# Ray0089/geometric-aware-dense-matching

Measured on AMD Instinct MI355X. Metric: rgbd_crops_per_sec_geomatch_fwd, higher is better.
Workload: dtype bf16x3/f32acc

## Files before the change

geometric_aware_dense_matching_amd/csrc/gdm_conv.hip:

```cpp
#include "gdm_common.h"
#include <math.h>
#include <limits.h>
#include <stdlib.h>

namespace {

constexpr int ROWB = 512;
constexpr int CV_PIX = 256;
constexpr int CV_CO = 128;
constexpr int CV_PANEL = CV_CO * ROWB;
#ifndef GDM_CONV16_PF
#define GDM_CONV16_PF 2
#endif

__device__ __forceinline__ void split8(const float* v, unsigned (&hi)[4], unsigned (&lo)[4])
{
#pragma unroll
    for (int j = 0; j < 4; ++j) gdm_split2(v[2 * j], v[2 * j + 1], hi[j], lo[j]);
}

__global__ __launch_bounds__(256) void conv_pack_act_kernel(const float* __restrict__ x, int C, int H, int W,
                                                            unsigned char* __restrict__ out)
{
    __shared__ float t[128][65];
// ... 57 lines not shown
#define GDM_CONV16_LATE 1
#endif
constexpr int MF_NPH = GDM_CONV_NPH;
constexpr int MF_WPIX = 16 * MF_NPH;
constexpr int MF_WAVES = CV_PIX / MF_WPIX;
constexpr int MF_THREADS = MF_WAVES * 64;
constexpr int conv_lds_bytes(int NCB)
{
    const int panels = 2 * NCB * 16 * ROWB, tiles = CV_PIX * (NCB * 16 + 4) * 4;
    return panels > tiles ? panels : tiles;
}
constexpr int LDS_MAX = 160 * 1024;
static_assert(conv_lds_bytes(8) == 135168 && conv_lds_bytes(4) == 69632 && conv_lds_bytes(9) == 151552 && conv_lds_bytes(8) >= 2 * CV_PANEL,
              "at least what every launch site passes");

template <int ACT, bool HAS_RES, int TAPS = 9, bool PIXMAJOR = false, int NKS = 8, int NCB = 8, int WV = MF_WAVES, bool GADD = false>
__global__ __launch_bounds__(MF_THREADS) void conv_mfma16_kernel(const unsigned char* __restrict__ xpk, const unsigned char* __restrict__ wpk,
                                                                 const float* __restrict__ scale, const float* __restrict__ shift,
                                                                 const float* __restrict__ res, int B, int Cin, int Cout, int H, int W,
                                                                 float* __restrict__ out, const int32_t* __restrict__ rowidx = nullptr,
                                                                 const int32_t* __restrict__ tile_co0 = nullptr,
                                                                 unsigned char* __restrict__ outpk = nullptr, int stride = 1,
                                                                 long wbstride = 0,
                                                                 const int32_t* __restrict__ gidx = nullptr,
                                                                 const float* __restrict__ gt = nullptr, int gn = 0,
                                                                 int gt_lds = 0)
{
    extern __shared__ __attribute__((aligned(16))) unsigned char smem[];
    constexpr int NS = NKS / 2;
    constexpr int UG = (NCB % 2 == 0) ? 2 : 3;
    constexpr int NPR = NCB / UG;
    constexpr int PANEL = NCB * 16 * ROWB;
    constexpr int TST = NCB * 16 + 4;
    static_assert(NCB == 8 || (NCB == 4 && !PIXMAJOR) || (NCB == 9 && !PIXMAJOR && WV == 8),
                  "64-channel tiles: NCHW / packed output only; 144-channel tiles: NCHW fp32 output only (no packed output: a tile straddles 128-channel chunks)");
    constexpr int NPH = MF_NPH;
    const int tid = threadIdx.x, lane = tid & 63;
    const int wave = __builtin_amdgcn_readfirstlane(tid >> 6);
    const int l16 = lane & 15, kg = lane >> 4;
    const int nchunk = (Cin + 127) / 128;
    const int npanel = TAPS * nchunk;
    const int hw = H * W;
    const long ptot = rowidx ? (long)B : (long)B * hw;
    const unsigned bx = blockIdx.x, by = blockIdx.y;
    const long pix0 = (long)bx * (WV * MF_WPIX) + wave * MF_WPIX;
    const int co0 = tile_co0 ? __builtin_amdgcn_readfirstlane(tile_co0[bx]) : by * (NCB * 16);
    const long pc = min(pix0, ptot - MF_WPIX);
    const int b = (int)(pc / hw);
    const int prem = (int)(pc - (long)b * hw);
    const int Wi = W * stride;
    const long plane = (long)(H * stride + 2) * (Wi + 2);
    const long oplane = (long)(H + 2) * (W + 2);
    const __amdgpu_buffer_rsrc_t xr = __builtin_amdgcn_make_buffer_rsrc(const_cast<unsigned char*>(xpk), (short)0, 0x7ffffff0, 0x00020000);
    int avoff[NPH];
#pragma unroll
    for (int ph = 0; ph < NPH; ++ph) {
        const int pr = prem + 16 * ph;
        const int yy = pr / W, xx = pr - yy * W;
        const long pixbase = rowidx ? (long)max(rowidx[pc + l16 + 16 * ph], 0) : (long)(yy * stride) * (Wi + 2) + (long)(xx + l16) * stride;
        avoff[ph] = (int)(((long)kg * plane + pixbase) * 16);
    }

    gdm_u32x4 ahi[NS][NPH], alo[NS][NPH];
    struct Pan { int chunk, ky, kx; };
    auto pan_next = [&](Pan p) -> Pan {
        if (TAPS == 1) { ++p.chunk; return p; }
        if (++p.kx == 3) { p.kx = 0; if (++p.ky == 3) { p.ky = 0; ++p.chunk; } }
        return p;
    };
    const int a_base = (int)(((long)(rowidx ? 0 : b) * nchunk * 32) * plane * 16);
    const int a_chunk = (int)(32 * plane * 16), a_rowb = (Wi + 2) * 16;
    auto pan_a = [&](Pan p) -> int { return a_base + p.chunk * a_chunk + p.ky * a_rowb + p.kx * 16; };
    const int sstride = (int)(4 * plane * 16);
    const int lostride = (int)(16 * plane * 16);
    auto load_a = [&](int r, int S) {
#pragma unroll
        for (int ph = 0; ph < NPH; ++ph) {
            ahi[S][ph] = __builtin_bit_cast(gdm_u32x4, __builtin_amdgcn_raw_buffer_load_b128(xr, avoff[ph], r + S * sstride, 0));
            alo[S][ph] = __builtin_bit_cast(gdm_u32x4, __builtin_amdgcn_raw_buffer_load_b128(xr, avoff[ph], r + S * sstride + lostride, 0));
        }
    };
    constexpr int THREADS = WV * 64, WGPIX = WV * MF_WPIX;
    constexpr int HS = (NCB * 512 / THREADS) / 2;
    gdm_u32x4 stage[HS];
    const __amdgpu_buffer_rsrc_t wr = __builtin_amdgcn_make_buffer_rsrc(const_cast<unsigned char*>(wpk), (short)0, 0x7ffffff0, 0x00020000);
    const int w_base = (wbstride ? (int)(((long)bx * WGPIX / hw) * wbstride) : 0) + co0 * ROWB;
    const int w_panel = ((Cout + 127) & ~127) * ROWB;
    auto pan_w = [&](Pan p) -> int { return w_base + ((TAPS == 1) ? p.chunk : (p.ky * 3 + p.kx) * nchunk + p.chunk) * w_panel; };
    auto stage_load = [&](int src, int half) {
#pragma unroll
        for (int i = 0; i < HS; ++i)
            stage[i] = __builtin_bit_cast(gdm_u32x4, __builtin_amdgcn_raw_buffer_load_b128(wr, tid * 16, src + (half * HS + i) * THREADS * 16, 0));
    };
    auto stage_store = [&](int buf, int half) {
        unsigned char* base = smem + buf * PANEL;
#pragma unroll
        for (int i = 0; i < HS; ++i) {
            const int g = (half * HS + i) * THREADS + tid;
            *reinterpret_cast<gdm_u32x4*>(base + gdm_swz<ROWB>(g >> 5, g & 31)) = stage[i];
        }
    };
    constexpr bool GLDS = WV == 8;
    constexpr int NPIECE = PANEL / 1024 / 8;
    int glds_voff = 0;
    if (GLDS) {
        const int hrow = lane >> 5, sl = lane & 31;
        const int col15 = (2 * wave + hrow) & 15;
        glds_voff = wave * 1024 + hrow * 512 + (((sl & 16) | ((sl ^ col15) & 15)) << 4);
    }
    typedef __attribute__((address_space(3))) void* lds_void_ptr;
    auto stage_glds = [&](int src, int buf) {
#pragma unroll
        for (int i = 0; i < NPIECE; ++i)
            __builtin_amdgcn_raw_ptr_buffer_load_lds(wr, (lds_void_ptr)(smem + buf * PANEL + (i * 8 + wave) * 1024), 16, glds_voff, src + i * 8192, 0, 0);
    };

    gdm_f32x4 acc[NPH][NCB];
#pragma unroll
    for (int ph = 0; ph < NPH; ++ph)
#pragma unroll
        for (int cb = 0; cb < NCB; ++cb)
#pragma unroll
            for (int i = 0; i < 4; ++i) acc[ph][cb][i] = 0.f;

    constexpr int LATE = GDM_CONV16_LATE < NS ? GDM_CONV16_LATE : NS;
    Pan pcur = {0, (TAPS == 1) ? 1 : 0, (TAPS == 1) ? 1 : 0};
    if (GLDS) {
        stage_glds(pan_w(pcur), 0);
    } else {
        stage_load(pan_w(pcur), 0);
        stage_store(0, 0);
        stage_load(pan_w(pcur), 1);
        stage_store(0, 1);
    }
    int rcur = pan_a(pcur);
#pragma unroll
    for (int S = 0; S < NS - LATE; ++S) load_a(rcur, S);
    Pan pnxt = npanel > 1 ? pan_next(pcur) : pcur;
    int rnext = pan_a(pnxt), wnext = pan_w(pnxt);
    for (int it = 0; it < npanel; ++it) {
        __syncthreads();
        const bool more = it + 1 < npanel;
        const unsigned char* base = smem + (it & 1) * PANEL;
        constexpr int PF = GDM_CONV16_PF;
        constexpr int NU = NPR * NS;
        gdm_u32x4 fh[PF + 1][UG], fl[PF + 1][UG];
        auto frag_load = [&](int un) {
            const int S = un / NPR, pr = un % NPR, slot = un % (PF + 1);
#pragma unroll
            for (int j = 0; j < UG; ++j) {
                const int col = (UG * pr + j) * 16 + l16;
                fh[slot][j] = *reinterpret_cast<const gdm_u32x4*>(base + gdm_swz<ROWB>(col, 4 * S + kg));
                fl[slot][j] = *reinterpret_cast<const gdm_u32x4*>(base + gdm_swz<ROWB>(col, 16 + 4 * S + kg));
            }
        };
#pragma unroll
        for (int un = 0; un < PF; ++un) frag_load(un);
#pragma unroll
        for (int u = 0; u < NU; ++u) {
            const int S = u / NPR, pr = u % NPR, slot = u % (PF + 1);
            if (u + PF < NU) frag_load(u + PF);
#pragma unroll
            for (int ph = 0; ph < NPH; ++ph) {
                const gdm_bf16x8 ah = __builtin_bit_cast(gdm_bf16x8, ahi[S][ph]);
                const gdm_bf16x8 al = __builtin_bit_cast(gdm_bf16x8, alo[S][ph]);
#pragma unroll
                for (int j = 0; j < UG; ++j) {
                    gdm_f32x4 c = acc[ph][UG * pr + j];
                    c = __builtin_amdgcn_mfma_f32_16x16x32_bf16(ah, __builtin_bit_cast(gdm_bf16x8, fl[slot][j]), c, 0, 0, 0);
                    c = __builtin_amdgcn_mfma_f32_16x16x32_bf16(al, __builtin_bit_cast(gdm_bf16x8, fh[slot][j]), c, 0, 0, 0);
                    c = __builtin_amdgcn_mfma_f32_16x16x32_bf16(ah, __builtin_bit_cast(gdm_bf16x8, fh[slot][j]), c, 0, 0, 0);
                    acc[ph][UG * pr + j] = c;
                }
            }
            if (pr == NPR - 1 && S < NS - LATE) load_a(rnext, S);
            if (!GLDS && u == NU / 2 && more) {
                stage_store((it + 1) & 1, 0);
                stage_load(wnext, 1);
            }
            if (u == 0) {
                if (more) { if (GLDS) stage_glds(wnext, (it + 1) & 1); else stage_load(wnext, 0); }
#pragma unroll
                for (int S2 = NS - LATE; S2 < NS; ++S2) load_a(rcur, S2);
            }
#pragma unroll
            for (int i = 0; i < 3 * UG * NPH; ++i) {
                __builtin_amdgcn_sched_group_barrier(0x008, 1, 0);
                if (u + PF < NU && (i % NPH) == 0 && i < 2 * UG * NPH) __builtin_amdgcn_sched_group_barrier(0x100, 1, 0);
            }
            __builtin_amdgcn_sched_barrier(0);
        }
        if (!GLDS && more) stage_store((it + 1) & 1, 1);
        rcur = rnext;
        if (it + 2 < npanel) pnxt = pan_next(pnxt);
        rnext = pan_a(pnxt);
        wnext = pan_w(pnxt);
    }

    if (pix0 >= ptot) return;
    if (PIXMAJOR) {
#pragma unroll
        for (int cb = 0; cb < NCB; ++cb) {
            const int co = co0 + cb * 16 + l16;
            if (co >= Cout) continue;
            const float sc = scale ? scale[co] : 1.f, sh = shift ? shift[co] : 0.f;
            const int ocol = tile_co0 ? cb * 16 + l16 : co;
            const int ostride = tile_co0 ? CV_CO : Cout;
#pragma unroll
            for (int ph = 0; ph < NPH; ++ph)
#pragma unroll
                for (int r = 0; r < 4; ++r) {
                    float v = acc[ph][cb][r] * sc + sh;
                    if (ACT == 1) v = fmaxf(v, 0.f);
                    out[(pix0 + 16 * ph + 4 * kg + r) * ostride + ocol] = v;
                }
        }
        return;
    }
    float gtv[GADD ? NPH : 1][GADD ? NCB : 1][4], gsc[GADD ? NCB : 1], gsh[GADD ? NCB : 1];
    int gsrc[GADD ? NPH : 1][4];
    if constexpr (GADD) {
#pragma unroll
        for (int ph = 0; ph < NPH; ++ph) {
            const int4 i4 = *reinterpret_cast<const int4*>(gidx + (long)b * hw + prem + 16 * ph + 4 * kg);
            gsrc[ph][0] = min(max(i4.x, 0), gn - 1);
            gsrc[ph][1] = min(max(i4.y, 0), gn - 1);
            gsrc[ph][2] = min(max(i4.z, 0), gn - 1);
            gsrc[ph][3] = min(max(i4.w, 0), gn - 1);
        }
#pragma unroll
        for (int cb = 0; cb < NCB; ++cb) {
            const int cl = min(co0 + cb * 16 + l16, Cout - 1);
            gsc[cb] = scale[cl];
            gsh[cb] = shift[cl];
        }
        if (gt_lds) {
            float* ts = reinterpret_cast<float*>(smem + gt_lds);
            for (int r = wave; r < NCB * 16; r += WV) {
                const float* tp = gt + ((long)b * Cout + min(co0 + r, Cout - 1)) * gn;
                for (int c = lane; c < gn; c += 64) ts[r * (gn + 1) + c] = tp[c];
            }
        } else {
#pragma unroll
            for (int cb = 0; cb < NCB; ++cb) {
                const float* tp = gt + ((long)b * Cout + min(co0 + cb * 16 + l16, Cout - 1)) * gn;
#pragma unroll
                for (int ph = 0; ph < NPH; ++ph)
#pragma unroll
                    for (int j = 0; j < 4; ++j) gtv[ph][cb][j] = tp[gsrc[ph][j]];
            }
        }
    }
    float* tl = reinterpret_cast<float*>(smem) + wave * MF_WPIX * TST;
    if (outpk || (GADD && gt_lds)) __syncthreads();
    if constexpr (GADD) {
        if (gt_lds) {
            const float* ts = reinterpret_cast<const float*>(smem + gt_lds);
#pragma unroll
            for (int cb = 0; cb < NCB; ++cb)
#pragma unroll
                for (int ph = 0; ph < NPH; ++ph)
#pragma unroll
                    for (int j = 0; j < 4; ++j) gtv[ph][cb][j] = ts[(cb * 16 + l16) * (gn + 1) + gsrc[ph][j]];
        }
    }
#pragma unroll
    for (int cb = 0; cb < NCB; ++cb) {
        const int co = co0 + cb * 16 + l16;
        const bool live = co < Cout;
        float sc, sh;
        if constexpr (GADD) { sc = gsc[cb]; sh = gsh[cb]; }
        else { sc = (live && scale) ? scale[co] : 1.f; sh = (live && shift) ? shift[co] : 0.f; }
        float* op = out ? out + ((long)b * Cout + (live ? co : 0)) * hw + prem : nullptr;
        const float* rp = (HAS_RES && live) ? res + ((long)b * Cout + co) * hw + prem : nullptr;
#pragma unroll
        for (int ph = 0; ph < NPH; ++ph) {
            const int poff = 16 * ph + 4 * kg;
            float v[4];
            if constexpr (GADD) {
#pragma unroll
                for (int j = 0; j < 4; ++j) {
                    const float x = acc[ph][cb][j] * 1.f + 0.f;
                    v[j] = (x + gtv[ph][cb][j]) * sc + sh;
                }
            } else {
#pragma unroll
                for (int j = 0; j < 4; ++j) v[j] = acc[ph][cb][j] * sc + sh;
            }
            if (HAS_RES && live) {
                const float4 r4 = *reinterpret_cast<const float4*>(rp + poff);
                v[0] += r4.x; v[1] += r4.y; v[2] += r4.z; v[3] += r4.w;
            }
            if (ACT == 1) {
#pragma unroll
                for (int j = 0; j < 4; ++j) v[j] = fmaxf(v[j], 0.f);
            }
            if (op && live) *reinterpret_cast<float4*>(op + poff) = make_float4(v[0], v[1], v[2], v[3]);
            if (outpk) {
#pragma unroll
                for (int j = 0; j < 4; ++j) tl[(poff + j) * TST + cb * 16 + l16] = live ? v[j] : 0.f;
            }
        }
    }
    if (outpk) {
        __builtin_amdgcn_fence(__ATOMIC_ACQ_REL, "wavefront");
        const int lr = lane & 31, h = lane >> 5;
        const int ochunks = (Cout + 127) / 128;
        const int ochunk = co0 / 128;
#pragma unroll
        for (int half = 0; half < MF_WPIX / 32; ++half) {
            const int pp = prem + 32 * half + lr;
            const int yy = pp / W, xx = pp - yy * W;
            unsigned char* ob = outpk + (((long)(b * ochunks + ochunk) * 32) * oplane + (long)(yy + 1) * (W + 2) + xx + 1) * 16;
            const float* row = tl + (32 * half + lr) * TST;
#pragma unroll
            for (int it = 0; it < NCB; ++it) {
                const int ql = 2 * it + h;
                if (co0 + ql * 8 >= Cout) continue;
                const int q = (co0 % 128) / 8 + ql;
                const float4 a0 = *reinterpret_cast<const float4*>(row + ql * 8);
                const float4 a1 = *reinterpret_cast<const float4*>(row + ql * 8 + 4);
                const float v[8] = {a0.x, a0.y, a0.z, a0.w, a1.x, a1.y, a1.z, a1.w};
                unsigned hi[4], lo[4];
                split8(v, hi, lo);
                *reinterpret_cast<uint4*>(ob + (long)q * oplane * 16) = make_uint4(hi[0], hi[1], hi[2], hi[3]);
                *reinterpret_cast<uint4*>(ob + (long)(16 + q) * oplane * 16) = make_uint4(lo[0], lo[1], lo[2], lo[3]);
            }
        }
    }
}

struct ConvArgs {
    const void *xpk = nullptr, *wpk = nullptr;
    const float *scale = nullptr, *shift = nullptr, *res = nullptr;
    int B = 0, Cin = 0, Cout = 0, H = 0, W = 0;
    float* out = nullptr;
    const int32_t *rowidx = nullptr, *tile_co0 = nullptr;
    void* outpk = nullptr;
    int stride = 1;
    long wbstride = 0;
    const int32_t* gidx = nullptr;
    const float* gt = nullptr;
    int gn = 0, gt_lds = 0;
    const char* who = "conv_mfma16_kernel";
};

static long mul_sat(long a, long b)
{
    long r;
    return (a < 0 || b < 0 || __builtin_mul_overflow(a, b, &r)) ? LONG_MAX : r;
}

template <int ACT, bool RES, int TAPS, bool PM, int NKS, int NCB, int WV, bool GADD>
int conv_launch(dim3 grid, int smem, hipStream_t s, const ConvArgs& a)
{
    const long chunks = (a.Cin + 127) / 128;
    const long xbytes = mul_sat(mul_sat(a.rowidx ? 1 : a.B, mul_sat((long)a.H * a.stride + 2, (long)a.W * a.stride + 2)), chunks * ROWB);
    const long wpanels = mul_sat(TAPS * chunks, (((long)a.Cout + 127) & ~127L) * ROWB);
    const long wlead = a.wbstride ? mul_sat(a.B - 1, a.wbstride) : 0;
    const long wbytes = wlead > LONG_MAX - wpanels ? LONG_MAX : wlead + wpanels;
    GDM_CHECK_ARG(xbytes < (1L << 31) && wbytes < (1L << 31),
                  "%s: packed operands must stay below 2 GiB (activations %ld bytes, weights %ld bytes)", a.who, xbytes, wbytes);
    GDM_CHECK_ARG((((uintptr_t)a.xpk | (uintptr_t)a.wpk) & 15) == 0,
                  "%s: the packed operands must be 16-byte aligned (xpk %p, wpk %p)", a.who, a.xpk, a.wpk);
    GDM_CHECK_ARG((((uintptr_t)a.res | (uintptr_t)a.out) & 15) == 0, "%s: res and out must be 16-byte aligned (res %p, out %p)", a.who,
                  (const void*)a.res, (const void*)a.out);
    constexpr auto kernel = conv_mfma16_kernel<ACT, RES, TAPS, PM, NKS, NCB, WV, GADD>;
    gdm_allow_lds<kernel>(GADD ? LDS_MAX : conv_lds_bytes(NCB));
    hipLaunchKernelGGL(kernel, grid, dim3(WV * 64), smem, s, (const unsigned char*)a.xpk, (const unsigned char*)a.wpk, a.scale, a.shift, a.res,
                       a.B, a.Cin, a.Cout, a.H, a.W, a.out, a.rowidx, a.tile_co0, (unsigned char*)a.outpk, a.stride, a.wbstride, a.gidx, a.gt,
                       a.gn, a.gt_lds);
    return 0;
}

}

namespace {
template <int CHAIN>
__global__ __launch_bounds__(512) void mfma_probe_kernel(int iters, float* __restrict__ sink)
{
    const int lane = threadIdx.x & 63;
    gdm_f32x4 acc[8];
#pragma unroll
    for (int i = 0; i < 8; ++i) acc[i] = gdm_f32x4{0.f, 0.f, 0.f, 0.f};
    const unsigned seed = 0x3f803f80u + (unsigned)lane;
    gdm_u32x4 av = {seed, seed ^ 1u, seed ^ 2u, seed ^ 3u}, bv = {seed ^ 4u, seed ^ 5u, seed ^ 6u, seed ^ 7u};
    const gdm_bf16x8 a = __builtin_bit_cast(gdm_bf16x8, av), b = __builtin_bit_cast(gdm_bf16x8, bv);
    for (int it = 0; it < iters; it += CHAIN) {
#pragma unroll
// ... 178 lines not shown
    return gdm_launch_status("gemm_grouped_kernel");
}

extern "C" int gdm_conv1x1_packed_wb_hip(const void* xpk, const void* wpk, long w_bstride, int B, int Cin, int Cout, int H, int W, float* out,
                                         void* stream)
{
    GDM_CHECK_ARG(xpk && wpk && out, "gdm_conv1x1_packed_wb_hip: NULL pointer");
    GDM_CHECK_ARG(B >= 1 && Cin >= 128 && Cin % 128 == 0 && Cout >= 1, "gdm_conv1x1_packed_wb_hip: Cin=%d Cout=%d (Cin a multiple of 128)", Cin, Cout);
    GDM_CHECK_ARG(W % 32 == 0 && H >= 1 && (H * W) % CV_PIX == 0, "gdm_conv1x1_packed_wb_hip: W=%d must be a multiple of 32 and H*W=%d of %d",
                  W, H * W, CV_PIX);
    GDM_CHECK_ARG(w_bstride >= 0 && w_bstride % 16 == 0, "gdm_conv1x1_packed_wb_hip: w_bstride=%ld", w_bstride);
    const long ptot = (long)B * H * W;
    const dim3 grid(gdm_cdiv(ptot, CV_PIX), gdm_cdiv(Cout, CV_CO));
    ConvArgs a{xpk, wpk, nullptr, nullptr, nullptr, B, Cin, Cout, H, W, out};
    a.wbstride = w_bstride; a.who = "gdm_conv1x1_packed_wb_hip";
    if (int refused = conv_launch<0, false, 1, false, 8, 8, MF_WAVES, false>(grid, 2 * CV_PANEL, (hipStream_t)stream, a)) return refused;
    return gdm_launch_status("conv1x1_bf16x3_kernel (per-image weights)");
}

static int conv1x1_launch(const void* xpk, const void* wpk, const float* scale, const float* shift,
                          int B, int Cin, int Cout, int H, int W, int stride, int act, int pixel_major, float* out, void* stream,
                          const char* who)
{
    GDM_CHECK_ARG(stride == 1 || stride == 2, "%s: stride=%d (1 or 2)", who, stride);
    GDM_CHECK_ARG(xpk && wpk && out, "%s: NULL pointer", who);
    GDM_CHECK_ARG(B >= 1 && cin_ok(Cin) && Cout >= 1, "%s: Cin=%d Cout=%d (Cin a multiple of 128, or 64)", who, Cin, Cout);
    GDM_CHECK_ARG(Cin != 64 || !pixel_major, "%s: Cin=64 is built for the NCHW output only", who);
    GDM_CHECK_ARG(W % 32 == 0 && H >= 1 && (H * W) % MF_WPIX == 0,
                  "%s: W=%d must be a multiple of 32 and H*W=%d of %d", who, W, H * W, MF_WPIX);
    GDM_CHECK_ARG(act == 0 || act == 1, "%s: act=%d", who, act);
    const long ptot = (long)B * H * W;
    const unsigned ptiles = gdm_cdiv(ptot, CV_PIX);
    hipStream_t s = (hipStream_t)stream;
    ConvArgs a{xpk, wpk, scale, shift, nullptr, B, Cin, Cout, H, W, out};
    a.stride = stride; a.who = who;
    int refused = 0;
    if (Cin != 64 && !pixel_major && stride == 1 && Cout % 144 == 0) {
        const long r128 = gdm_cdiv((long)ptiles * gdm_cdiv(Cout, 128), 256) * 128, r144 = gdm_cdiv((long)ptiles * (Cout / 144), 256) * 144;
        if (r144 < r128) {
            const dim3 grid9(ptiles, Cout / 144);
            gdm_dispatch_int<2>(act, [&](auto A) {
                refused = conv_launch<decltype(A)::value, false, 1, false, 8, 9, MF_WAVES, false>(grid9, conv_lds_bytes(9), s, a);
            });
            if (refused) return refused;
            return gdm_launch_status("conv1x1_bf16x3_kernel (144-channel tiles)");
        }
    }
    const bool narrow = Cin != 64 && !pixel_major && narrow_tiles(ptiles, Cout);
    const unsigned ctiles = gdm_cdiv(Cout, narrow ? 64 : CV_CO);
    const dim3 grid(ptiles, ctiles);
    gdm_dispatch_int<2>(act, [&](auto A) {
        constexpr int ACT = decltype(A)::value;
        if (Cin == 64)
            refused = conv_launch<ACT, false, 1, false, 4, 8, MF_WAVES, false>(grid, 2 * CV_PANEL, s, a);
        else if (narrow)
            refused = conv_launch<ACT, false, 1, false, 8, 4, MF_WAVES, false>(grid, 2 * 64 * ROWB, s, a);
        else
            gdm_dispatch_bool(pixel_major != 0, [&](auto P) {
                refused = conv_launch<ACT, false, 1, decltype(P)::value, 8, 8, MF_WAVES, false>(grid, 2 * CV_PANEL, s, a);
            });
    });
    if (refused) return refused;
    return gdm_launch_status(narrow ? "conv1x1_bf16x3_kernel (64-channel tiles)" : "conv1x1_bf16x3_kernel");
}

extern "C" int gdm_conv1x1_packed_hip(const void* xpk, const void* wpk, const float* scale, const float* shift,
                                      int B, int Cin, int Cout, int H, int W, int act, int pixel_major, float* out, void* stream)
{
    return conv1x1_launch(xpk, wpk, scale, shift, B, Cin, Cout, H, W, 1, act, pixel_major, out, stream, "gdm_conv1x1_packed_hip");
}

extern "C" int gdm_conv1x1_strided_hip(const void* xpk, const void* wpk, const float* scale, const float* shift,
                                       int B, int Cin, int Cout, int H, int W, int stride, int act, float* out, void* stream)
{
// ... 38 lines not shown
```

include/gdm.h:

```cpp
#ifndef GDM_H
#define GDM_H

#include <stddef.h>
#include <stdint.h>

#ifdef __cplusplus
extern "C" {
#endif

#define GDM_EINVAL (-1)
#define GDM_ENOMEM (-2)

const char* gdm_last_error(void);
int gdm_version(void);


void gdm_knn_batch(const float* batch_data, size_t batch_size, size_t npts, size_t dim,
                   const float* queries, size_t nqueries, size_t K, long* batch_indices);

int gdm_knn_batch_hip(const float* support, const float* query, int B, int S, int Q, int K,
                      int32_t* idx, float* d2, void* stream);

typedef struct gdm_knn_job {
    const float* support;
// ... 321 lines not shown
int gdm_stem_hip(const float* x, const void* wpk, const float* scale, const float* shift, int B, int H, int W, float* out,
                 void* out_packed, void* stream);

size_t gdm_wgrad_x_bytes(int B, int Cin, int H, int W);
size_t gdm_wgrad_go_bytes(int B, int Cout, int H, int W);
int gdm_wgrad_pack_x_hip(const float* x, int B, int Cin, int H, int W, void* out, void* stream);
int gdm_wgrad_pack_go_hip(const float* go, int B, int Cout, int H, int W, void* out, void* stream);
size_t gdm_wgrad_x1_bytes(int B, int Cin, int P);
int gdm_wgrad_pack_x1_hip(const float* x, int B, int Cin, int P, void* out, void* stream);
int gdm_mfma_probe_hip(int blocks, int iters, int chain, float* sink, void* stream);
int gdm_mfma_probe_lds_hip(int blocks, int iters, int rpu, float* sink, void* stream);
int gdm_wgrad_direct_hip(const float* go, long go_bstride, const float* x, long x_bstride, int B, int Cout, int Cin, int P,
                         int nsplit, float* partial, float* bias_partial, void* stream);
int gdm_conv1x1_packed_wb_hip(const void* xpk, const void* wpk, long w_bstride, int B, int Cin, int Cout, int H, int W, float* out,
                              void* stream);

typedef struct gdm_copy_job {
    void* dst;
    const void* src;
    int64_t sb, s1, s2;
    int32_t B, R1, R2, E;
} gdm_copy_job;
#define GDM_COPY_MAX_JOBS 16
int gdm_copy_jobs_hip(const gdm_copy_job* jobs , int njobs, void* stream);

int gdm_mssd_mspd_hip(const double* RT_est, const double* RT_gt, const double* pts, const double* sym_R, const double* sym_t,
                      const double* K, int k_per_instance, int n, int M, int S, double* err, double* mssd, double* mspd,
                      int32_t* best_sym_mssd, int32_t* best_sym_mspd, void* stream);
int gdm_render_depth_hip(const void* verts, int verts_f64, const int32_t* faces, const double* RT, const double* K, int k_per_instance,
                         int n, int V, int F, int H, int W, double near, int keep_inf, float* depth, void* stream);
// ... 25 lines not shown
```

Before: 5271.

## Make 1x1 conv kernels persistent, prefetching the next tile's operands across tiles

The 1x1 MFMA conv sites now launch a persistent grid sized to CU count times workgroups per CU. Each workgroup loops over output tiles with a grid stride. While finishing the last panel of one tile, it prefetches the next tile's activation fragments and weight panel, so the pipeline fill is not paid per tile and launch/tail overhead drops. In exchange there are fewer workgroups in flight, more register pressure from the extra tile state, and a possible load imbalance at the tail.

```diff
diff --git a/geometric_aware_dense_matching_amd/csrc/gdm_conv.hip b/geometric_aware_dense_matching_amd/csrc/gdm_conv.hip
--- a/geometric_aware_dense_matching_amd/csrc/gdm_conv.hip
+++ b/geometric_aware_dense_matching_amd/csrc/gdm_conv.hip
@@ -2,6 +2,7 @@
 #include <math.h>
 #include <limits.h>
 #include <stdlib.h>
+#include <atomic>
 
 namespace {
 
@@ -95,7 +96,8 @@
 static_assert(conv_lds_bytes(8) == 135168 && conv_lds_bytes(4) == 69632 && conv_lds_bytes(9) == 151552 && conv_lds_bytes(8) >= 2 * CV_PANEL,
               "at least what every launch site passes");
 
-template <int ACT, bool HAS_RES, int TAPS = 9, bool PIXMAJOR = false, int NKS = 8, int NCB = 8, int WV = MF_WAVES, bool GADD = false>
+template <int ACT, bool HAS_RES, int TAPS = 9, bool PIXMAJOR = false, int NKS = 8, int NCB = 8, int WV = MF_WAVES, bool GADD = false,
+          bool LOOP = false>
 __global__ __launch_bounds__(MF_THREADS) void conv_mfma16_kernel(const unsigned char* __restrict__ xpk, const unsigned char* __restrict__ wpk,
                                                                  const float* __restrict__ scale, const float* __restrict__ shift,
                                                                  const float* __restrict__ res, int B, int Cin, int Cout, int H, int W,
@@ -105,8 +107,10 @@
                                                                  long wbstride = 0,
                                                                  const int32_t* __restrict__ gidx = nullptr,
                                                                  const float* __restrict__ gt = nullptr, int gn = 0,
-                                                                 int gt_lds = 0)
-{
+                                                                 int gt_lds = 0,
+                                                                 unsigned ntiles = 0, unsigned ptiles = 1)
+{
+    static_assert(!LOOP || (TAPS == 1 && WV == 8 && !GADD), "the tile loop is built for the plain 1x1 sites: one tap, weight panels by LDS-DMA");
     extern __shared__ __attribute__((aligned(16))) unsigned char smem[];
     constexpr int NS = NKS / 2;
     constexpr int UG = (NCB % 2 == 0) ? 2 : 3;
@@ -123,24 +127,43 @@
     const int npanel = TAPS * nchunk;
     const int hw = H * W;
     const long ptot = rowidx ? (long)B : (long)B * hw;
-    const unsigned bx = blockIdx.x, by = blockIdx.y;
-    const long pix0 = (long)bx * (WV * MF_WPIX) + wave * MF_WPIX;
-    const int co0 = tile_co0 ? __builtin_amdgcn_readfirstlane(tile_co0[bx]) : by * (NCB * 16);
-    const long pc = min(pix0, ptot - MF_WPIX);
-    const int b = (int)(pc / hw);
-    const int prem = (int)(pc - (long)b * hw);
     const int Wi = W * stride;
     const long plane = (long)(H * stride + 2) * (Wi + 2);
     const long oplane = (long)(H + 2) * (W + 2);
+    constexpr int THREADS = WV * 64, WGPIX = WV * MF_WPIX;
+    struct Tile {
+        long pix0;
+        int co0, b, prem;
+        int a_base, w_base;
+        int avoff[NPH];
+    };
+    auto tile_at = [&](unsigned bx, unsigned by) -> Tile {
+        Tile T;
+        T.pix0 = (long)bx * WGPIX + wave * MF_WPIX;
+        T.co0 = tile_co0 ? __builtin_amdgcn_readfirstlane(tile_co0[bx]) : by * (NCB * 16);
+        const long pc = min(T.pix0, ptot - MF_WPIX);
+        T.b = (int)(pc / hw);
+        T.prem = (int)(pc - (long)T.b * hw);
+#pragma unroll
+        for (int ph = 0; ph < NPH; ++ph) {
+            const int pr = T.prem + 16 * ph;
+            const int yy = pr / W, xx = pr - yy * W;
+            const long pixbase = rowidx ? (long)max(rowidx[pc + l16 + 16 * ph], 0) : (long)(yy * stride) * (Wi + 2) + (long)(xx + l16) * stride;
+            T.avoff[ph] = (int)(((long)kg * plane + pixbase) * 16);
+        }
+        T.a_base = (int)(((long)(rowidx ? 0 : T.b) * nchunk * 32) * plane * 16);
+        T.w_base = (wbstride ? (int)(((long)bx * WGPIX / hw) * wbstride) : 0) + T.co0 * ROWB;
+        return T;
+    };
+    unsigned t = blockIdx.x;
+    auto next_of = [&](unsigned tt) -> unsigned { return tt + gridDim.x < ntiles ? tt + gridDim.x : tt; };
+    Tile cur = LOOP ? tile_at(t % ptiles, t / ptiles) : tile_at(blockIdx.x, blockIdx.y);
+    unsigned tn = LOOP ? next_of(t) : t;
+    Tile nxt_tile = LOOP ? tile_at(tn % ptiles, tn / ptiles) : Tile{};
+    Tile& nxt = LOOP ? nxt_tile : cur;
+    const long& pix0 = cur.pix0;
+    const int &co0 = cur.co0, &b = cur.b, &prem = cur.prem;
     const __amdgpu_buffer_rsrc_t xr = __builtin_amdgcn_make_buffer_rsrc(const_cast<unsigned char*>(xpk), (short)0, 0x7ffffff0, 0x00020000);
-    int avoff[NPH];
-#pragma unroll
-    for (int ph = 0; ph < NPH; ++ph) {
-        const int pr = prem + 16 * ph;
-        const int yy = pr / W, xx = pr - yy * W;
-        const long pixbase = rowidx ? (long)max(rowidx[pc + l16 + 16 * ph], 0) : (long)(yy * stride) * (Wi + 2) + (long)(xx + l16) * stride;
-        avoff[ph] = (int)(((long)kg * plane + pixbase) * 16);
-    }
 
     gdm_u32x4 ahi[NS][NPH], alo[NS][NPH];
     struct Pan { int chunk, ky, kx; };
@@ -149,25 +172,22 @@
         if (++p.kx == 3) { p.kx = 0; if (++p.ky == 3) { p.ky = 0; ++p.chunk; } }
         return p;
     };
-    const int a_base = (int)(((long)(rowidx ? 0 : b) * nchunk * 32) * plane * 16);
     const int a_chunk = (int)(32 * plane * 16), a_rowb = (Wi + 2) * 16;
-    auto pan_a = [&](Pan p) -> int { return a_base + p.chunk * a_chunk + p.ky * a_rowb + p.kx * 16; };
+    auto pan_a = [&](const Tile& T, Pan p) -> int { return T.a_base + p.chunk * a_chunk + p.ky * a_rowb + p.kx * 16; };
     const int sstride = (int)(4 * plane * 16);
     const int lostride = (int)(16 * plane * 16);
-    auto load_a = [&](int r, int S) {
+    auto load_a = [&](const int* avoff, int r, int S) {
 #pragma unroll
         for (int ph = 0; ph < NPH; ++ph) {
             ahi[S][ph] = __builtin_bit_cast(gdm_u32x4, __builtin_amdgcn_raw_buffer_load_b128(xr, avoff[ph], r + S * sstride, 0));
             alo[S][ph] = __builtin_bit_cast(gdm_u32x4, __builtin_amdgcn_raw_buffer_load_b128(xr, avoff[ph], r + S * sstride + lostride, 0));
         }
     };
-    constexpr int THREADS = WV * 64, WGPIX = WV * MF_WPIX;
     constexpr int HS = (NCB * 512 / THREADS) / 2;
     gdm_u32x4 stage[HS];
     const __amdgpu_buffer_rsrc_t wr = __builtin_amdgcn_make_buffer_rsrc(const_cast<unsigned char*>(wpk), (short)0, 0x7ffffff0, 0x00020000);
-    const int w_base = (wbstride ? (int)(((long)bx * WGPIX / hw) * wbstride) : 0) + co0 * ROWB;
     const int w_panel = ((Cout + 127) & ~127) * ROWB;
-    auto pan_w = [&](Pan p) -> int { return w_base + ((TAPS == 1) ? p.chunk : (p.ky * 3 + p.kx) * nchunk + p.chunk) * w_panel; };
+    auto pan_w = [&](const Tile& T, Pan p) -> int { return T.w_base + ((TAPS == 1) ? p.chunk : (p.ky * 3 + p.kx) * nchunk + p.chunk) * w_panel; };
     auto stage_load = [&](int src, int half) {
 #pragma unroll
         for (int i = 0; i < HS; ++i)
@@ -197,216 +217,236 @@
     };
 
     gdm_f32x4 acc[NPH][NCB];
-#pragma unroll
-    for (int ph = 0; ph < NPH; ++ph)
-#pragma unroll
-        for (int cb = 0; cb < NCB; ++cb)
-#pragma unroll
-            for (int i = 0; i < 4; ++i) acc[ph][cb][i] = 0.f;
-
     constexpr int LATE = GDM_CONV16_LATE < NS ? GDM_CONV16_LATE : NS;
-    Pan pcur = {0, (TAPS == 1) ? 1 : 0, (TAPS == 1) ? 1 : 0};
+    const Pan pfirst = {0, (TAPS == 1) ? 1 : 0, (TAPS == 1) ? 1 : 0};
     if (GLDS) {
-        stage_glds(pan_w(pcur), 0);
+        stage_glds(pan_w(cur, pfirst), 0);
     } else {
-        stage_load(pan_w(pcur), 0);
+        stage_load(pan_w(cur, pfirst), 0);
         stage_store(0, 0);
-        stage_load(pan_w(pcur), 1);
+        stage_load(pan_w(cur, pfirst), 1);
         stage_store(0, 1);
     }
-    int rcur = pan_a(pcur);
-#pragma unroll
-    for (int S = 0; S < NS - LATE; ++S) load_a(rcur, S);
-    Pan pnxt = npanel > 1 ? pan_next(pcur) : pcur;
-    int rnext = pan_a(pnxt), wnext = pan_w(pnxt);
-    for (int it = 0; it < npanel; ++it) {
-        __syncthreads();
-        const bool more = it + 1 < npanel;
-        const unsigned char* base = smem + (it & 1) * PANEL;
-        constexpr int PF = GDM_CONV16_PF;
-        constexpr int NU = NPR * NS;
-        gdm_u32x4 fh[PF + 1][UG], fl[PF + 1][UG];
-        auto frag_load = [&](int un) {
-            const int S = un / NPR, pr = un % NPR, slot = un % (PF + 1);
-#pragma unroll
-            for (int j = 0; j < UG; ++j) {
-                const int col = (UG * pr + j) * 16 + l16;
-                fh[slot][j] = *reinterpret_cast<const gdm_u32x4*>(base + gdm_swz<ROWB>(col, 4 * S + kg));
-                fl[slot][j] = *reinterpret_cast<const gdm_u32x4*>(base + gdm_swz<ROWB>(col, 16 + 4 * S + kg));
+#pragma unroll
+    for (int S = 0; S < NS - LATE; ++S) load_a(cur.avoff, pan_a(cur, pfirst), S);
+    unsigned pcnt = 0;
+    for (;;) {
+        const bool last_tile = !LOOP || tn == t;
+#pragma unroll
+        for (int ph = 0; ph < NPH; ++ph)
+#pragma unroll
+            for (int cb = 0; cb < NCB; ++cb)
+#pragma unroll
+                for (int i = 0; i < 4; ++i) acc[ph][cb][i] = 0.f;
+        int rcur = pan_a(cur, pfirst);
+        Pan pnxt = npanel > 1 ? pan_next(pfirst) : pfirst;
+        int rnext = (LOOP && npanel == 1) ? pan_a(nxt, pfirst) : pan_a(cur, pnxt);
+        int wnext = (LOOP && npanel == 1) ? pan_w(nxt, pfirst) : pan_w(cur, pnxt);
+        for (int it = 0; it < npanel; ++it, ++pcnt) {
+            __syncthreads();
+            const bool more = it + 1 < npanel;
+            const bool wmore = more || !last_tile;
+            const unsigned char* base = smem + (pcnt & 1) * PANEL;
+            int avnext[NPH];
+#pragma unroll
+            for (int ph = 0; ph < NPH; ++ph) avnext[ph] = (LOOP && !more) ? nxt.avoff[ph] : cur.avoff[ph];
+            constexpr int PF = GDM_CONV16_PF;
+            constexpr int NU = NPR * NS;
+            gdm_u32x4 fh[PF + 1][UG], fl[PF + 1][UG];
+            auto frag_load = [&](int un) {
+                const int S = un / NPR, pr = un % NPR, slot = un % (PF + 1);
+#pragma unroll
+                for (int j = 0; j < UG; ++j) {
+                    const int col = (UG * pr + j) * 16 + l16;
+                    fh[slot][j] = *reinterpret_cast<const gdm_u32x4*>(base + gdm_swz<ROWB>(col, 4 * S + kg));
+                    fl[slot][j] = *reinterpret_cast<const gdm_u32x4*>(base + gdm_swz<ROWB>(col, 16 + 4 * S + kg));
+                }
+            };
+#pragma unroll
+            for (int un = 0; un < PF; ++un) frag_load(un);
+#pragma unroll
+            for (int u = 0; u < NU; ++u) {
+                const int S = u / NPR, pr = u % NPR, slot = u % (PF + 1);
+                if (u + PF < NU) frag_load(u + PF);
+#pragma unroll
+                for (int ph = 0; ph < NPH; ++ph) {
+                    const gdm_bf16x8 ah = __builtin_bit_cast(gdm_bf16x8, ahi[S][ph]);
+                    const gdm_bf16x8 al = __builtin_bit_cast(gdm_bf16x8, alo[S][ph]);
+#pragma unroll
+                    for (int j = 0; j < UG; ++j) {
+                        gdm_f32x4 c = acc[ph][UG * pr + j];
+                        c = __builtin_amdgcn_mfma_f32_16x16x32_bf16(ah, __builtin_bit_cast(gdm_bf16x8, fl[slot][j]), c, 0, 0, 0);
+                        c = __builtin_amdgcn_mfma_f32_16x16x32_bf16(al, __builtin_bit_cast(gdm_bf16x8, fh[slot][j]), c, 0, 0, 0);
+                        c = __builtin_amdgcn_mfma_f32_16x16x32_bf16(ah, __builtin_bit_cast(gdm_bf16x8, fh[slot][j]), c, 0, 0, 0);
+                        acc[ph][UG * pr + j] = c;
+                    }
+                }
+                if (pr == NPR - 1 && S < NS - LATE) load_a(avnext, rnext, S);
+                if (!GLDS && u == NU / 2 && more) {
+                    stage_store((pcnt + 1) & 1, 0);
+                    stage_load(wnext, 1);
+                }
+                if (u == 0) {
+                    if (wmore) { if (GLDS) stage_glds(wnext, (pcnt + 1) & 1); else stage_load(wnext, 0); }
+#pragma unroll
+                    for (int S2 = NS - LATE; S2 < NS; ++S2) load_a(cur.avoff, rcur, S2);
+                }
+#pragma unroll
+                for (int i = 0; i < 3 * UG * NPH; ++i) {
+                    __builtin_amdgcn_sched_group_barrier(0x008, 1, 0);
+                    if (u + PF < NU && (i % NPH) == 0 && i < 2 * UG * NPH) __builtin_amdgcn_sched_group_barrier(0x100, 1, 0);
+                }
+                __builtin_amdgcn_sched_barrier(0);
             }
-        };
-#pragma unroll
-        for (int un = 0; un < PF; ++un) frag_load(un);
-#pragma unroll
-        for (int u = 0; u < NU; ++u) {
-            const int S = u / NPR, pr = u % NPR, slot = u % (PF + 1);
-            if (u + PF < NU) frag_load(u + PF);
-#pragma unroll
-            for (int ph = 0; ph < NPH; ++ph) {
-                const gdm_bf16x8 ah = __builtin_bit_cast(gdm_bf16x8, ahi[S][ph]);
-                const gdm_bf16x8 al = __builtin_bit_cast(gdm_bf16x8, alo[S][ph]);
-#pragma unroll
-                for (int j = 0; j < UG; ++j) {
-                    gdm_f32x4 c = acc[ph][UG * pr + j];
-                    c = __builtin_amdgcn_mfma_f32_16x16x32_bf16(ah, __builtin_bit_cast(gdm_bf16x8, fl[slot][j]), c, 0, 0, 0);
-                    c = __builtin_amdgcn_mfma_f32_16x16x32_bf16(al, __builtin_bit_cast(gdm_bf16x8, fh[slot][j]), c, 0, 0, 0);
-                    c = __builtin_amdgcn_mfma_f32_16x16x32_bf16(ah, __builtin_bit_cast(gdm_bf16x8, fh[slot][j]), c, 0, 0, 0);
-                    acc[ph][UG * pr + j] = c;
-                }
-            }
-            if (pr == NPR - 1 && S < NS - LATE) load_a(rnext, S);
-            if (!GLDS && u == NU / 2 && more) {
-                stage_store((it + 1) & 1, 0);
-                stage_load(wnext, 1);
-            }
-            if (u == 0) {
-                if (more) { if (GLDS) stage_glds(wnext, (it + 1) & 1); else stage_load(wnext, 0); }
-#pragma unroll
-                for (int S2 = NS - LATE; S2 < NS; ++S2) load_a(rcur, S2);
-            }
-#pragma unroll
-            for (int i = 0; i < 3 * UG * NPH; ++i) {
-                __builtin_amdgcn_sched_group_barrier(0x008, 1, 0);
-                if (u + PF < NU && (i % NPH) == 0 && i < 2 * UG * NPH) __builtin_amdgcn_sched_group_barrier(0x100, 1, 0);
-            }
-            __builtin_amdgcn_sched_barrier(0);
+            if (!GLDS && more) stage_store((pcnt + 1) & 1, 1);
+            rcur = rnext;
+            if (it + 2 < npanel) pnxt = pan_next(pnxt);
+            const bool over = LOOP && it + 2 >= npanel;
+            rnext = over ? pan_a(nxt, pfirst) : pan_a(cur, pnxt);
+            wnext = over ? pan_w(nxt, pfirst) : pan_w(cur, pnxt);
         }
-        if (!GLDS && more) stage_store((it + 1) & 1, 1);
-        rcur = rnext;
-        if (it + 2 < npanel) pnxt = pan_next(pnxt);
-        rnext = pan_a(pnxt);
-        wnext = pan_w(pnxt);
-    }
-
-    if (pix0 >= ptot) return;
-    if (PIXMAJOR) {
-#pragma unroll
-        for (int cb = 0; cb < NCB; ++cb) {
-            const int co = co0 + cb * 16 + l16;
-            if (co >= Cout) continue;
-            const float sc = scale ? scale[co] : 1.f, sh = shift ? shift[co] : 0.f;
-            const int ocol = tile_co0 ? cb * 16 + l16 : co;
-            const int ostride = tile_co0 ? CV_CO : Cout;
-#pragma unroll
-            for (int ph = 0; ph < NPH; ++ph)
-#pragma unroll
-                for (int r = 0; r < 4; ++r) {
-                    float v = acc[ph][cb][r] * sc + sh;
-                    if (ACT == 1) v = fmaxf(v, 0.f);
-                    out[(pix0 + 16 * ph + 4 * kg + r) * ostride + ocol] = v;
-                }
-        }
-        return;
-    }
-    float gtv[GADD ? NPH : 1][GADD ? NCB : 1][4], gsc[GADD ? NCB : 1], gsh[GADD ? NCB : 1];
-    int gsrc[GADD ? NPH : 1][4];
-    if constexpr (GADD) {
-#pragma unroll
-        for (int ph = 0; ph < NPH; ++ph) {
-            const int4 i4 = *reinterpret_cast<const int4*>(gidx + (long)b * hw + prem + 16 * ph + 4 * kg);
-            gsrc[ph][0] = min(max(i4.x, 0), gn - 1);
-            gsrc[ph][1] = min(max(i4.y, 0), gn - 1);
-            gsrc[ph][2] = min(max(i4.z, 0), gn - 1);
-            gsrc[ph][3] = min(max(i4.w, 0), gn - 1);
-        }
-#pragma unroll
-        for (int cb = 0; cb < NCB; ++cb) {
-            const int cl = min(co0 + cb * 16 + l16, Cout - 1);
-            gsc[cb] = scale[cl];
-            gsh[cb] = shift[cl];
-        }
-        if (gt_lds) {
-            float* ts = reinterpret_cast<float*>(smem + gt_lds);
-            for (int r = wave; r < NCB * 16; r += WV) {
-                const float* tp = gt + ((long)b * Cout + min(co0 + r, Cout - 1)) * gn;
-                for (int c = lane; c < gn; c += 64) ts[r * (gn + 1) + c] = tp[c];
+
+        if (!LOOP && pix0 >= ptot) return;
+        const bool wlive = !LOOP || pix0 < ptot;
+        int lane = tid & 63;
+        if constexpr (LOOP) asm volatile("" : "+v"(lane));
+        const int l16 = lane & 15, kg = lane >> 4;
+        if constexpr (PIXMAJOR) {
+#pragma unroll
+            for (int cb = 0; cb < NCB; ++cb) {
+                const int co = co0 + cb * 16 + l16;
+                if (co >= Cout) continue;
+                const float sc = scale ? scale[co] : 1.f, sh = shift ? shift[co] : 0.f;
+                const int ocol = tile_co0 ? cb * 16 + l16 : co;
+                const int ostride = tile_co0 ? CV_CO : Cout;
+#pragma unroll
+                for (int ph = 0; ph < NPH; ++ph)
+#pragma unroll
+                    for (int r = 0; r < 4; ++r) {
+                        float v = acc[ph][cb][r] * sc + sh;
+                        if (ACT == 1) v = fmaxf(v, 0.f);
+                        if (wlive) out[(pix0 + 16 * ph + 4 * kg + r) * ostride + ocol] = v;
+                    }
             }
         } else {
+            float gtv[GADD ? NPH : 1][GADD ? NCB : 1][4], gsc[GADD ? NCB : 1], gsh[GADD ? NCB : 1];
+            int gsrc[GADD ? NPH : 1][4];
+            if constexpr (GADD) {
+#pragma unroll
+                for (int ph = 0; ph < NPH; ++ph) {
+                    const int4 i4 = *reinterpret_cast<const int4*>(gidx + (long)b * hw + prem + 16 * ph + 4 * kg);
+                    gsrc[ph][0] = min(max(i4.x, 0), gn - 1);
+                    gsrc[ph][1] = min(max(i4.y, 0), gn - 1);
+                    gsrc[ph][2] = min(max(i4.z, 0), gn - 1);
+                    gsrc[ph][3] = min(max(i4.w, 0), gn - 1);
+                }
+#pragma unroll
+                for (int cb = 0; cb < NCB; ++cb) {
+                    const int cl = min(co0 + cb * 16 + l16, Cout - 1);
+                    gsc[cb] = scale[cl];
+                    gsh[cb] = shift[cl];
+                }
+                if (gt_lds) {
+                    float* ts = reinterpret_cast<float*>(smem + gt_lds);
+                    for (int r = wave; r < NCB * 16; r += WV) {
+                        const float* tp = gt + ((long)b * Cout + min(co0 + r, Cout - 1)) * gn;
+                        for (int c = lane; c < gn; c += 64) ts[r * (gn + 1) + c] = tp[c];
+                    }
+                } else {
+#pragma unroll
+                    for (int cb = 0; cb < NCB; ++cb) {
+                        const float* tp = gt + ((long)b * Cout + min(co0 + cb * 16 + l16, Cout - 1)) * gn;
+#pragma unroll
+                        for (int ph = 0; ph < NPH; ++ph)
+#pragma unroll
+                            for (int j = 0; j < 4; ++j) gtv[ph][cb][j] = tp[gsrc[ph][j]];
+                    }
+                }
+            }
+            float* tl = reinterpret_cast<float*>(smem) + wave * MF_WPIX * TST;
+            if (outpk || (GADD && gt_lds)) __syncthreads();
+            if constexpr (GADD) {
+                if (gt_lds) {
+                    const float* ts = reinterpret_cast<const float*>(smem + gt_lds);
+#pragma unroll
+                    for (int cb = 0; cb < NCB; ++cb)
+#pragma unroll
+                        for (int ph = 0; ph < NPH; ++ph)
+#pragma unroll
+                            for (int j = 0; j < 4; ++j) gtv[ph][cb][j] = ts[(cb * 16 + l16) * (gn + 1) + gsrc[ph][j]];
+                }
+            }
 #pragma unroll
             for (int cb = 0; cb < NCB; ++cb) {
-                const float* tp = gt + ((long)b * Cout + min(co0 + cb * 16 + l16, Cout - 1)) * gn;
-#pragma unroll
-                for (int ph = 0; ph < NPH; ++ph)
-#pragma unroll
-                    for (int j = 0; j < 4; ++j) gtv[ph][cb][j] = tp[gsrc[ph][j]];
+                const int co = co0 + cb * 16 + l16;
+                const bool live = co < Cout;
+                float sc, sh;
+                if constexpr (GADD) { sc = gsc[cb]; sh = gsh[cb]; }
+                else { sc = (live && scale) ? scale[co] : 1.f; sh = (live && shift) ? shift[co] : 0.f; }
+                float* op = out ? out + ((long)b * Cout + (live ? co : 0)) * hw + prem : nullptr;
+                const float* rp = (HAS_RES && live) ? res + ((long)b * Cout + co) * hw + prem : nullptr;
+#pragma unroll
+                for (int ph = 0; ph < NPH; ++ph) {
+                    const int poff = 16 * ph + 4 * kg;
+                    float v[4];
+                    if constexpr (GADD) {
+#pragma unroll
+                        for (int j = 0; j < 4; ++j) {
+                            const float x = acc[ph][cb][j] * 1.f + 0.f;
+                            v[j] = (x + gtv[ph][cb][j]) * sc + sh;
+                        }
+                    } else {
+#pragma unroll
+                        for (int j = 0; j < 4; ++j) v[j] = acc[ph][cb][j] * sc + sh;
+                    }
+                    if (HAS_RES && live) {
+                        const float4 r4 = *reinterpret_cast<const float4*>(rp + poff);
+                        v[0] += r4.x; v[1] += r4.y; v[2] += r4.z; v[3] += r4.w;
+                    }
+                    if (ACT == 1) {
+#pragma unroll
+                        for (int j = 0; j < 4; ++j) v[j] = fmaxf(v[j], 0.f);
+                    }
+                    if (op && live && wlive) *reinterpret_cast<float4*>(op + poff) = make_float4(v[0], v[1], v[2], v[3]);
+                    if (outpk) {
+#pragma unroll
+                        for (int j = 0; j < 4; ++j) tl[(poff + j) * TST + cb * 16 + l16] = live ? v[j] : 0.f;
+                    }
+                }
+            }
+            if (outpk && wlive) {
+                __builtin_amdgcn_fence(__ATOMIC_ACQ_REL, "wavefront");
+                const int lr = lane & 31, h = lane >> 5;
+                const int ochunks = (Cout + 127) / 128;
+                const int ochunk = co0 / 128;
+#pragma unroll
+                for (int half = 0; half < MF_WPIX / 32; ++half) {
+                    const int pp = prem + 32 * half + lr;
+                    const int yy = pp / W, xx = pp - yy * W;
+                    unsigned char* ob = outpk + (((long)(b * ochunks + ochunk) * 32) * oplane + (long)(yy + 1) * (W + 2) + xx + 1) * 16;
+                    const float* row = tl + (32 * half + lr) * TST;
+#pragma unroll
+                    for (int it = 0; it < NCB; ++it) {
+                        const int ql = 2 * it + h;
+                        if (co0 + ql * 8 >= Cout) continue;
+                        const int q = (co0 % 128) / 8 + ql;
+                        const float4 a0 = *reinterpret_cast<const float4*>(row + ql * 8);
+                        const float4 a1 = *reinterpret_cast<const float4*>(row + ql * 8 + 4);
+                        const float v[8] = {a0.x, a0.y, a0.z, a0.w, a1.x, a1.y, a1.z, a1.w};
+                        unsigned hi[4], lo[4];
+                        split8(v, hi, lo);
+                        *reinterpret_cast<uint4*>(ob + (long)q * oplane * 16) = make_uint4(hi[0], hi[1], hi[2], hi[3]);
+                        *reinterpret_cast<uint4*>(ob + (long)(16 + q) * oplane * 16) = make_uint4(lo[0], lo[1], lo[2], lo[3]);
+                    }
+                }
             }
         }
-    }
-    float* tl = reinterpret_cast<float*>(smem) + wave * MF_WPIX * TST;
-    if (outpk || (GADD && gt_lds)) __syncthreads();
-    if constexpr (GADD) {
-        if (gt_lds) {
-            const float* ts = reinterpret_cast<const float*>(smem + gt_lds);
-#pragma unroll
-            for (int cb = 0; cb < NCB; ++cb)
-#pragma unroll
-                for (int ph = 0; ph < NPH; ++ph)
-#pragma unroll
-                    for (int j = 0; j < 4; ++j) gtv[ph][cb][j] = ts[(cb * 16 + l16) * (gn + 1) + gsrc[ph][j]];
-        }
-    }
-#pragma unroll
-    for (int cb = 0; cb < NCB; ++cb) {
-        const int co = co0 + cb * 16 + l16;
-        const bool live = co < Cout;
-        float sc, sh;
-        if constexpr (GADD) { sc = gsc[cb]; sh = gsh[cb]; }
-        else { sc = (live && scale) ? scale[co] : 1.f; sh = (live && shift) ? shift[co] : 0.f; }
-        float* op = out ? out + ((long)b * Cout + (live ? co : 0)) * hw + prem : nullptr;
-        const float* rp = (HAS_RES && live) ? res + ((long)b * Cout + co) * hw + prem : nullptr;
-#pragma unroll
-        for (int ph = 0; ph < NPH; ++ph) {
-            const int poff = 16 * ph + 4 * kg;
-            float v[4];
-            if constexpr (GADD) {
-#pragma unroll
-                for (int j = 0; j < 4; ++j) {
-                    const float x = acc[ph][cb][j] * 1.f + 0.f;
-                    v[j] = (x + gtv[ph][cb][j]) * sc + sh;
-                }
-            } else {
-#pragma unroll
-                for (int j = 0; j < 4; ++j) v[j] = acc[ph][cb][j] * sc + sh;
-            }
-            if (HAS_RES && live) {
-                const float4 r4 = *reinterpret_cast<const float4*>(rp + poff);
-                v[0] += r4.x; v[1] += r4.y; v[2] += r4.z; v[3] += r4.w;
-            }
-            if (ACT == 1) {
-#pragma unroll
-                for (int j = 0; j < 4; ++j) v[j] = fmaxf(v[j], 0.f);
-            }
-            if (op && live) *reinterpret_cast<float4*>(op + poff) = make_float4(v[0], v[1], v[2], v[3]);
-            if (outpk) {
-#pragma unroll
-                for (int j = 0; j < 4; ++j) tl[(poff + j) * TST + cb * 16 + l16] = live ? v[j] : 0.f;
-            }
-        }
-    }
-    if (outpk) {
-        __builtin_amdgcn_fence(__ATOMIC_ACQ_REL, "wavefront");
-        const int lr = lane & 31, h = lane >> 5;
-        const int ochunks = (Cout + 127) / 128;
-        const int ochunk = co0 / 128;
-#pragma unroll
-        for (int half = 0; half < MF_WPIX / 32; ++half) {
-            const int pp = prem + 32 * half + lr;
-            const int yy = pp / W, xx = pp - yy * W;
-            unsigned char* ob = outpk + (((long)(b * ochunks + ochunk) * 32) * oplane + (long)(yy + 1) * (W + 2) + xx + 1) * 16;
-            const float* row = tl + (32 * half + lr) * TST;
-#pragma unroll
-            for (int it = 0; it < NCB; ++it) {
-                const int ql = 2 * it + h;
-                if (co0 + ql * 8 >= Cout) continue;
-                const int q = (co0 % 128) / 8 + ql;
-                const float4 a0 = *reinterpret_cast<const float4*>(row + ql * 8);
-                const float4 a1 = *reinterpret_cast<const float4*>(row + ql * 8 + 4);
-                const float v[8] = {a0.x, a0.y, a0.z, a0.w, a1.x, a1.y, a1.z, a1.w};
-                unsigned hi[4], lo[4];
-                split8(v, hi, lo);
-                *reinterpret_cast<uint4*>(ob + (long)q * oplane * 16) = make_uint4(hi[0], hi[1], hi[2], hi[3]);
-                *reinterpret_cast<uint4*>(ob + (long)(16 + q) * oplane * 16) = make_uint4(lo[0], lo[1], lo[2], lo[3]);
-            }
+        if (last_tile) break;
+        if constexpr (LOOP) {
+            t = tn;
+            cur = nxt;
+            tn = next_of(t);
+            nxt = tile_at(tn % ptiles, tn / ptiles);
         }
     }
 }
@@ -424,7 +464,26 @@
     const float* gt = nullptr;
     int gn = 0, gt_lds = 0;
     const char* who = "conv_mfma16_kernel";
+    int wg_per_cu = 1;
 };
+
+std::atomic<int> g_tile_grid_cap{0};
+
+int conv_n_cu(int* n_cu)
+{
+    constexpr int MAXDEV = 64;
+    static std::atomic<int> known[MAXDEV];
+    int dev = 0;
+    GDM_HIP(hipGetDevice(&dev));
+    int n = (dev >= 0 && dev < MAXDEV) ? known[dev].load(std::memory_order_relaxed) : 0;
+    if (n == 0) {
+        GDM_HIP(hipDeviceGetAttribute(&n, hipDeviceAttributeMultiprocessorCount, dev));
+        GDM_CHECK_ARG(n >= 1, "conv_mfma16_kernel: device %d reports %d CUs", dev, n);
+        if (dev >= 0 && dev < MAXDEV) known[dev].store(n, std::memory_order_relaxed);
+    }
+    *n_cu = n;
+    return 0;
+}
 
 static long mul_sat(long a, long b)
 {
@@ -432,7 +491,7 @@
     return (a < 0 || b < 0 || __builtin_mul_overflow(a, b, &r)) ? LONG_MAX : r;
 }
 
-template <int ACT, bool RES, int TAPS, bool PM, int NKS, int NCB, int WV, bool GADD>
+template <int ACT, bool RES, int TAPS, bool PM, int NKS, int NCB, int WV, bool GADD, bool LOOP = false>
 int conv_launch(dim3 grid, int smem, hipStream_t s, const ConvArgs& a)
 {
     const long chunks = (a.Cin + 127) / 128;
@@ -446,14 +505,36 @@
                   "%s: the packed operands must be 16-byte aligned (xpk %p, wpk %p)", a.who, a.xpk, a.wpk);
     GDM_CHECK_ARG((((uintptr_t)a.res | (uintptr_t)a.out) & 15) == 0, "%s: res and out must be 16-byte aligned (res %p, out %p)", a.who,
                   (const void*)a.res, (const void*)a.out);
-    constexpr auto kernel = conv_mfma16_kernel<ACT, RES, TAPS, PM, NKS, NCB, WV, GADD>;
+    GDM_CHECK_ARG(!LOOP || !a.outpk, "%s: the tile loop writes fp32 output only", a.who);
+    constexpr auto kernel = conv_mfma16_kernel<ACT, RES, TAPS, PM, NKS, NCB, WV, GADD, LOOP>;
+    const unsigned ntiles = grid.x * grid.y, ptiles = grid.x;
+    if constexpr (LOOP) {
+        int n_cu = 0;
+        if (int rc = conv_n_cu(&n_cu)) return rc;
+        grid = dim3(gdm_conv_tile_grid(ntiles, n_cu, a.wg_per_cu, g_tile_grid_cap.load(std::memory_order_relaxed)));
+    }
     gdm_allow_lds<kernel>(GADD ? LDS_MAX : conv_lds_bytes(NCB));
     hipLaunchKernelGGL(kernel, grid, dim3(WV * 64), smem, s, (const unsigned char*)a.xpk, (const unsigned char*)a.wpk, a.scale, a.shift, a.res,
                        a.B, a.Cin, a.Cout, a.H, a.W, a.out, a.rowidx, a.tile_co0, (unsigned char*)a.outpk, a.stride, a.wbstride, a.gidx, a.gt,
-                       a.gn, a.gt_lds);
+                       a.gn, a.gt_lds, ntiles, ptiles);
     return 0;
 }
 
+}
+
+extern "C" int gdm_conv_tile_grid(long ntiles, int n_cu, int wg_per_cu, int cap)
+{
+    long g = (long)(n_cu > 1 ? n_cu : 1) * (wg_per_cu > 1 ? wg_per_cu : 1);
+    if (ntiles < g) g = ntiles;
+    if (cap > 0 && cap < g) g = cap;
+    return (int)(g > 1 ? g : 1);
+}
+
+extern "C" int gdm_conv_set_tile_grid_cap(int cap)
+{
+    GDM_CHECK_ARG(cap >= 0, "gdm_conv_set_tile_grid_cap: cap=%d (0 = no cap, or a positive number of workgroups)", cap);
+    g_tile_grid_cap.store(cap, std::memory_order_relaxed);
+    return 0;
 }
 
 namespace {
@@ -662,7 +743,7 @@
     const dim3 grid(gdm_cdiv(ptot, CV_PIX), gdm_cdiv(Cout, CV_CO));
     ConvArgs a{xpk, wpk, nullptr, nullptr, nullptr, B, Cin, Cout, H, W, out};
     a.wbstride = w_bstride; a.who = "gdm_conv1x1_packed_wb_hip";
-    if (int refused = conv_launch<0, false, 1, false, 8, 8, MF_WAVES, false>(grid, 2 * CV_PANEL, (hipStream_t)stream, a)) return refused;
+    if (int refused = conv_launch<0, false, 1, false, 8, 8, MF_WAVES, false, true>(grid, 2 * CV_PANEL, (hipStream_t)stream, a)) return refused;
     return gdm_launch_status("conv1x1_bf16x3_kernel (per-image weights)");
 }
 
@@ -688,7 +769,7 @@
         if (r144 < r128) {
             const dim3 grid9(ptiles, Cout / 144);
             gdm_dispatch_int<2>(act, [&](auto A) {
-                refused = conv_launch<decltype(A)::value, false, 1, false, 8, 9, MF_WAVES, false>(grid9, conv_lds_bytes(9), s, a);
+                refused = conv_launch<decltype(A)::value, false, 1, false, 8, 9, MF_WAVES, false, true>(grid9, conv_lds_bytes(9), s, a);
             });
             if (refused) return refused;
             return gdm_launch_status("conv1x1_bf16x3_kernel (144-channel tiles)");
@@ -697,15 +778,16 @@
     const bool narrow = Cin != 64 && !pixel_major && narrow_tiles(ptiles, Cout);
     const unsigned ctiles = gdm_cdiv(Cout, narrow ? 64 : CV_CO);
     const dim3 grid(ptiles, ctiles);
+    a.wg_per_cu = narrow ? 2 : 1;
     gdm_dispatch_int<2>(act, [&](auto A) {
         constexpr int ACT = decltype(A)::value;
         if (Cin == 64)
-            refused = conv_launch<ACT, false, 1, false, 4, 8, MF_WAVES, false>(grid, 2 * CV_PANEL, s, a);
+            refused = conv_launch<ACT, false, 1, false, 4, 8, MF_WAVES, false, true>(grid, 2 * CV_PANEL, s, a);
         else if (narrow)
-            refused = conv_launch<ACT, false, 1, false, 8, 4, MF_WAVES, false>(grid, 2 * 64 * ROWB, s, a);
+            refused = conv_launch<ACT, false, 1, false, 8, 4, MF_WAVES, false, true>(grid, 2 * 64 * ROWB, s, a);
         else
             gdm_dispatch_bool(pixel_major != 0, [&](auto P) {
-                refused = conv_launch<ACT, false, 1, decltype(P)::value, 8, 8, MF_WAVES, false>(grid, 2 * CV_PANEL, s, a);
+                refused = conv_launch<ACT, false, 1, decltype(P)::value, 8, 8, MF_WAVES, false, true>(grid, 2 * CV_PANEL, s, a);
             });
     });
     if (refused) return refused;
diff --git a/include/gdm.h b/include/gdm.h
--- a/include/gdm.h
+++ b/include/gdm.h
@@ -359,6 +359,8 @@
                          int nsplit, float* partial, float* bias_partial, void* stream);
 int gdm_conv1x1_packed_wb_hip(const void* xpk, const void* wpk, long w_bstride, int B, int Cin, int Cout, int H, int W, float* out,
                               void* stream);
+int gdm_conv_tile_grid(long ntiles, int n_cu, int wg_per_cu, int cap);
+int gdm_conv_set_tile_grid_cap(int cap);
 
 typedef struct gdm_copy_job {
     void* dst;
```

After: 5300, median of 6. No clear change (+0.6%).
